# VIPL-Audio-Visual-Speech-Understanding/SBL_For_Multilingual_Lip_Reading

Hardware: AMD Instinct MI355X
Metric: lip-clips/sec fwd+bwd (29x88x88) (higher is better)
Workload: dtype f32 (exact 3-way bf16 split, 6 bf16 MFMA products per fp32 product, fp32 accumulate); 1 GPU; full SBL 6+6 (Conv3d stem + ResNet-18 + encoder + SBL decoder) fwd+loss+bwd (BASELINE config 3); matmul_precision=bf16x6, per_gpu_batch=32, global_batch=32, clip=29x88x88, parallelism=dp1, dropout=True, bn=train, issue=graph, hipgraph=True, decoder_streams=2, conv_weight_pack=cached (re-packed when weights change), decoder_schedule=teacher-forced runs batched, coin_patterns=8

## Files before the change

sbl_for_multilingual_lip_reading_amd/csrc/gemm.hip:

```cpp
#include <stdarg.h>
#include <stdlib.h>

#include <type_traits>
#include "mfma_gemm.h"
#include "skinny_gemm.h"

static thread_local char g_err[512] = "";
void sbl_set_error(const char* fmt, ...) {
    va_list ap;
    va_start(ap, fmt);
    vsnprintf(g_err, sizeof(g_err), fmt, ap);
    va_end(ap);
}
extern "C" const char* sbl_last_error(void) { return g_err; }

static unsigned long long* g_stamps = nullptr;
static int g_stamp_cap = 0, g_stamp_used = 0;
static thread_local int g_last_slot = -1, g_last_kid = 0;
unsigned long long* sbl_next_stamp_slot(int kernel_id) {
    g_last_kid = kernel_id;
    g_last_slot = -1;
    if (!g_stamps || g_stamp_used >= g_stamp_cap) return nullptr;
    g_last_slot = g_stamp_used++;
    return g_stamps + 2 * (size_t)g_last_slot;
}
extern "C" int sbl_profile_begin(uint64_t* stamps_dev, int capacity) {
    SBL_REQUIRE(stamps_dev && capacity > 0, "sbl_profile_begin: bad args");
    g_stamps = (unsigned long long*)stamps_dev;
    g_stamp_cap = capacity;
    g_stamp_used = 0;
    return 0;
}
extern "C" int sbl_profile_end(void) {
    const int used = g_stamp_used;
    g_stamps = nullptr;
    g_stamp_cap = g_stamp_used = 0;
    return used;
}
extern "C" int sbl_profile_last_slot(void) { return g_last_slot; }
extern "C" int sbl_profile_used(void) { return g_stamp_used; }
extern "C" int sbl_profile_last_kernel(void) { return g_last_kid; }
extern "C" int sbl_abi_version(void) { return SBL_ABI_VERSION; }

int g_sbl_prec = 0;
extern "C" int sbl_set_matmul_precision(int terms) {
    SBL_REQUIRE(terms == 0 || terms == 1 || terms == 3 || terms == 6,
                "sbl_set_matmul_precision: %d (0 = fp32 MFMA, 6 / 3 / 1 = split-bf16 MFMA terms)", terms);
    g_sbl_prec = terms;
    return 0;
}
extern "C" int sbl_get_matmul_precision(void) { return g_sbl_prec; }
int g_sbl_exp[8] = {0, 0, 0, 0, 0, 0, 0, 0};
int g_sbl_gemm2_split_target = 256, g_sbl_gemm2_split_max = 8;
int g_sbl_group_cap = 0;
int g_sbl_wave_ksplit = 1;
int g_sbl_ksplit_tiles = 320;
int g_sbl_big_min = 4096;
extern "C" int sbl_set_tuning(int knob, int value) {
    extern int g_sbl_wg_s2_small, g_sbl_wg_target, g_sbl_conv_patch;
    if (knob >= 100 && knob < 108) {
        g_sbl_exp[knob - 100] = value;
        return 0;
    }
    if (knob == 14) {
        extern int g_sbl_stem_fwd8;
        g_sbl_stem_fwd8 = value != 0;
        return 0;
    }
    if (knob == 13) {
        extern int g_sbl_stem_ablate;
        g_sbl_stem_ablate = value;
        return 0;
    }
    if (knob == 12) {
        extern int g_sbl_stem_wgrad_tr;
        g_sbl_stem_wgrad_tr = value != 0;
        return 0;
    }
    if (knob == 10 || knob == 11) {
        SBL_REQUIRE(value >= 1, "sbl_set_tuning: value < 1");
        (knob == 10 ? g_sbl_gemm2_split_target : g_sbl_gemm2_split_max) = value;
        return 0;
    }
    if (knob == 9) {
        extern int g_sbl_conv_patch_wgrad;
        SBL_REQUIRE(value >= 0, "sbl_set_tuning: negative value");
        g_sbl_conv_patch_wgrad = value;
        return 0;
    }
    if (knob == 8) {
        extern int g_sbl_conv_patch_imgs;
        SBL_REQUIRE(value >= 0, "sbl_set_tuning: negative value");
        g_sbl_conv_patch_imgs = value;
        return 0;
    }
    if (knob == 7) {
        extern int g_sbl_pm_wg64_maxm;
        SBL_REQUIRE(value >= 0, "sbl_set_tuning: negative value");
        g_sbl_pm_wg64_maxm = value;
        return 0;
    }
    if (knob == 6) {
        SBL_REQUIRE(value >= 0, "sbl_set_tuning: negative value");
        g_sbl_group_cap = value;
        return 0;
    }
    if (knob >= 3 && knob <= 5) {
        SBL_REQUIRE(value >= 0, "sbl_set_tuning: negative value");
        (knob == 3 ? g_sbl_wg_s2_small : knob == 4 ? g_sbl_wg_target : g_sbl_conv_patch) = value;
        return 0;
    }
    SBL_REQUIRE(knob >= 0 && knob <= 2 && value >= 0, "sbl_set_tuning: unknown knob %d / value %d (0 = wave-group K split on/off, 1 = 64x64-tile count from which dense products take 128x128 tiles, 2 = largest tile count that takes the wave-group K split)", knob, value);
    if (knob == 0) g_sbl_wave_ksplit = value != 0;
    else if (knob == 1) g_sbl_big_min = value;
    else g_sbl_ksplit_tiles = value;
    return 0;
}

template <class AL, class BL, int BM, int BN, int KU>
static void launch_mode(const AL& al, const BL& bl, float* C, long ldc, const float* bias, int relu,
                        const float* relu_mask, long ldm, int mode, int M, int N, int K, int splits, SplitCtl sc,
                        hipStream_t s) {
    if (mode == 0) {
        EpiStore<0, false> e{C, ldc, bias, relu, nullptr, relu_mask, ldm};
        sbl_launch_gemm<AL, BL, EpiStore<0, false>, BM, BN, KU>(al, bl, e, M, N, K, splits, s, sc);
    } else if (mode == 1) {
        EpiStore<1, false> e{C, ldc, bias, relu, nullptr, relu_mask, ldm};
        sbl_launch_gemm<AL, BL, EpiStore<1, false>, BM, BN, KU>(al, bl, e, M, N, K, splits, s, sc);
    } else {
        EpiStore<2, false> e{C, ldc, nullptr, 0, nullptr, nullptr, 0};
        sbl_launch_gemm<AL, BL, EpiStore<2, false>, BM, BN, KU>(al, bl, e, M, N, K, splits, s, sc);
    }
}

template <bool VEC, int BM, int BN, int KU>
static void launch_trans(int transA, int transB, const float* A, long lda, const float* B, long ldb, float* C, long ldc,
                         const float* bias, int relu, const float* relu_mask, long ldm, int mode, int M, int N, int K,
                         int splits, SplitCtl sc, hipStream_t s) {
    if (!transA && transB) {
        DenseKC<BM, VEC> al{A, lda, M};
        DenseKC<BN, VEC> bl{B, ldb, N};
        launch_mode<DenseKC<BM, VEC>, DenseKC<BN, VEC>, BM, BN, KU>(al, bl, C, ldc, bias, relu, relu_mask, ldm, mode, M, N, K, splits, sc, s);
    } else if (!transA && !transB) {
        DenseKC<BM, VEC> al{A, lda, M};
        DenseMC<BN, VEC> bl{B, ldb, N};
        launch_mode<DenseKC<BM, VEC>, DenseMC<BN, VEC>, BM, BN, KU>(al, bl, C, ldc, bias, relu, relu_mask, ldm, mode, M, N, K, splits, sc, s);
    } else if (transA && !transB) {
        DenseMC<BM, VEC> al{A, lda, M};
        DenseMC<BN, VEC> bl{B, ldb, N};
        launch_mode<DenseMC<BM, VEC>, DenseMC<BN, VEC>, BM, BN, KU>(al, bl, C, ldc, bias, relu, relu_mask, ldm, mode, M, N, K, splits, sc, s);
    } else {
        DenseMC<BM, VEC> al{A, lda, M};
        DenseKC<BN, VEC> bl{B, ldb, N};
        launch_mode<DenseMC<BM, VEC>, DenseKC<BN, VEC>, BM, BN, KU>(al, bl, C, ldc, bias, relu, relu_mask, ldm, mode, M, N, K, splits, sc, s);
    }
}

#define SBL_WS_COUNTERS 4096

extern "C" int sbl_gemm_f32(int transA, int transB, int M, int N, int K, const float* A, long lda, const float* B,
                            long ldb, float* C, long ldc, const float* bias, int relu, const float* relu_mask, long ldm,
                            int accumulate, float* a_colsum, void* ws, long ws_bytes, sbl_stream_t stream) {
    hipStream_t s = (hipStream_t)stream;
    SBL_REQUIRE(M > 0 && N > 0 && K > 0, "sbl_gemm_f32: non-positive dims M=%d N=%d K=%d", M, N, K);
    SBL_REQUIRE(A && B && C, "sbl_gemm_f32: null operand");
    SBL_REQUIRE(lda >= (transA ? M : K) && ldb >= (transB ? K : N) && ldc >= N,
                "sbl_gemm_f32: leading dimension too small (lda=%ld ldb=%ld ldc=%ld)", lda, ldb, ldc);
    SBL_REQUIRE(!relu_mask || ldm >= N, "sbl_gemm_f32: ldm=%ld < N=%d", ldm, N);
    SBL_REQUIRE(!a_colsum || transA, "sbl_gemm_f32: a_colsum needs transA=1 (A stored [K][M])");
    SBL_REQUIRE(!ws || (sbl_aligned16(ws) && ws_bytes >= (long)sizeof(int) * SBL_WS_COUNTERS), "sbl_gemm_f32: workspace unaligned or < 16 KiB");
    bool vec = sbl_aligned16(A) && sbl_aligned16(B) && (lda % 4 == 0) && (ldb % 4 == 0);
    if (!transA || transB) vec = vec && (K % 4 == 0);
    if (transA) vec = vec && (M % 4 == 0);
    if (!transB) vec = vec && (N % 4 == 0);
    SBL_REQUIRE(sbl_fits_u32((transA ? (long)K : (long)M) * lda) && sbl_fits_u32((transB ? (long)N : (long)K) * ldb),
                "sbl_gemm_f32: operand spans more than 2 GiB (buffer descriptor range)");
    const bool plain = !bias && !relu && !relu_mask;
    const long tiles64 = (long)sbl_cdiv(M, 64) * sbl_cdiv(N, 64);
    const int big_min = g_sbl_big_min;
    const bool big = (M >= 1024 && N >= 256 && tiles64 >= big_min);
    int splits = 1;
    constexpr int split_tiles = 192;
    constexpr int split_target = 256;
    if (!big && tiles64 < split_tiles && K >= 128) {
        splits = (int)((split_target + tiles64 - 1) / tiles64);
        if (splits > K / 64) splits = K / 64;
        if (splits > 8) splits = 8;
        if (splits < 1) splits = 1;
    }
    SplitCtl sc{nullptr, nullptr, a_colsum, nullptr};
    int mode = accumulate ? 1 : 0;
    if (splits > 1) {
        const long need = (long)sizeof(int) * SBL_WS_COUNTERS + tiles64 * splits * (long)(64 * 64 * sizeof(float));
        if (ws && tiles64 < SBL_WS_COUNTERS && need <= ws_bytes) {
            sc.counters = (int*)ws;
            sc.slabs = (float*)((char*)ws + sizeof(int) * SBL_WS_COUNTERS);
        } else if (plain) {
            mode = 2;
            if (!accumulate) SBL_HIP(hipMemset2DAsync(C, ldc * sizeof(float), 0, (size_t)N * sizeof(float), M, s));
        } else {
            splits = 1;
        }
    }
    {
        const bool a_kc = !transA, b_kc = transB != 0;
        const bool al_ok = (!a_kc || (sbl_aligned16(A) && lda % 4 == 0)) && (!b_kc || (sbl_aligned16(B) && ldb % 4 == 0));
        const bool k_ok = (!a_kc && !b_kc) || (K % 8 == 0);
        const long tiles32 = (long)sbl_cdiv(M, 32) * sbl_cdiv(N, 32);
        constexpr int max_m = 512;
        constexpr int max_t = 2048;
        constexpr int sq_rows = 1536;
        const bool shape_ok = transA ? ((K <= max_m && tiles32 <= max_t) || ((long)M * N <= 512L * 512 && K <= sq_rows))
                                     : ((M <= max_m && tiles32 <= max_t) || ((long)N * K <= 512L * 512 && M <= sq_rows));
        if (shape_ok && al_ok && k_ok && !(transA && transB)) {
            SkinnyEpi e{C, ldc, bias, relu, relu_mask, ldm, accumulate, a_colsum, sbl_next_stamp_slot(SBL_KID_SKINNY)};
            if (!transA && transB) sbl_launch_skinny<true, true>(A, lda, B, ldb, e, M, N, K, s);
            else if (!transA && !transB) sbl_launch_skinny<true, false>(A, lda, B, ldb, e, M, N, K, s);
            else sbl_launch_skinny<false, false>(A, lda, B, ldb, e, M, N, K, s);
            SBL_LAUNCH_CHECK("sbl_gemm_f32(skinny)");
            return 0;
        }
    }
    sc.stamp = sbl_next_stamp_slot(big ? SBL_KID_TILED128 : SBL_KID_TILED64);
#define SBL_GO(VEC, BM, BN, KU) \
    launch_trans<VEC, BM, BN, KU>(transA, transB, A, lda, B, ldb, C, ldc, bias, relu, relu_mask, ldm, mode, M, N, K, splits, sc, s)
    if (big) {
        constexpr int big_ku = 1;
        if (vec && big_ku == 2) SBL_GO(true, 128, 128, 2);
        else if (vec) SBL_GO(true, 128, 128, 1);
        else SBL_GO(false, 128, 128, 1);
    } else {
        constexpr int ku_env = 0;
        const int ku = ku_env ? ku_env : (tiles64 * splits > 512 ? 2 : 4);
        if (!vec) SBL_GO(false, 64, 64, 1);
        else if (ku == 1) SBL_GO(true, 64, 64, 1);
        else if (ku == 2) SBL_GO(true, 64, 64, 2);
        else SBL_GO(true, 64, 64, 4);
    }
#undef SBL_GO
    SBL_LAUNCH_CHECK("sbl_gemm_f32");
    return 0;
}

extern "C" int sbl_gemm2_f32(int M, int N, int K, const float* A0, const float* A1, long lda, const float* B0, const float* B1,
                             long ldb, float* C0, float* C1, long ldc, const float* bias0, const float* bias1, int relu,
                             void* ws, long ws_bytes, sbl_stream_t stream) {
    hipStream_t s = (hipStream_t)stream;
    SBL_REQUIRE(M > 0 && N > 0 && K > 0, "sbl_gemm2_f32: non-positive dims M=%d N=%d K=%d", M, N, K);
    SBL_REQUIRE(A0 && A1 && B0 && B1 && C0 && C1 && (!bias0 == !bias1), "sbl_gemm2_f32: null operand / one-sided bias");
    SBL_REQUIRE(lda >= K && ldb >= K && ldc >= N, "sbl_gemm2_f32: leading dimension too small (lda=%ld ldb=%ld ldc=%ld)", lda, ldb, ldc);
    SBL_REQUIRE(!ws || (sbl_aligned16(ws) && ws_bytes >= (long)sizeof(int) * SBL_WS_COUNTERS), "sbl_gemm2_f32: workspace unaligned or < 16 KiB");
    const bool vec = sbl_aligned16(A0) && sbl_aligned16(A1) && sbl_aligned16(B0) && sbl_aligned16(B1) && lda % 4 == 0 && ldb % 4 == 0 && K % 8 == 0;
    SBL_REQUIRE(sbl_fits_u32((long)M * lda) && sbl_fits_u32((long)N * ldb), "sbl_gemm2_f32: operand spans more than 2 GiB (buffer descriptor range)");
    const long tiles64 = (long)sbl_cdiv(M, 64) * sbl_cdiv(N, 64);
    const int big_min = g_sbl_big_min;
    const bool big = (M >= 1024 && N >= 256 && 2 * tiles64 >= big_min);
    if (!vec || big) {
        if (int e = sbl_gemm_f32(0, 1, M, N, K, A0, lda, B0, ldb, C0, ldc, bias0, relu, nullptr, 0, 0, nullptr, ws, ws_bytes, stream)) return e;
        return sbl_gemm_f32(0, 1, M, N, K, A1, lda, B1, ldb, C1, ldc, bias1, relu, nullptr, 0, 0, nullptr, ws, ws_bytes, stream);
    }
    {
        const long tiles32 = (long)sbl_cdiv(M, 32) * sbl_cdiv(N, 32);
        constexpr int max_m = 128;
        constexpr int max_t = 2048;
        constexpr int sq_rows = 768;
        if ((M <= max_m && tiles32 <= max_t) || ((long)N * K <= 512L * 512 && M <= sq_rows)) {
            SkinnyEpi e{C0, ldc, bias0, relu, nullptr, 0, 0, nullptr, sbl_next_stamp_slot(SBL_KID_SKINNY)};
            SkinnyDual du{A1, B1, C1, bias1};
            sbl_launch_skinny<true, true>(A0, lda, B0, ldb, e, M, N, K, s, &du);
            SBL_LAUNCH_CHECK("sbl_gemm2_f32(skinny)");
            return 0;
        }
    }
    int splits = 1;
    const int split_tiles = g_sbl_exp[1] > 0 ? g_sbl_exp[1] : 192;
    const int split_target = g_sbl_gemm2_split_target;
    if (2 * tiles64 < split_tiles && K >= 128) {
        splits = (int)((split_target + 2 * tiles64 - 1) / (2 * tiles64));
        if (splits > K / 64) splits = K / 64;
        if (splits > g_sbl_gemm2_split_max) splits = g_sbl_gemm2_split_max;
        if (splits < 1) splits = 1;
    }
    SplitCtl sc{nullptr, nullptr, nullptr, nullptr};
    if (splits > 1) {
        const long need = (long)sizeof(int) * SBL_WS_COUNTERS + 2 * tiles64 * splits * (long)(64 * 64 * sizeof(float));
        if (ws && 2 * tiles64 < SBL_WS_COUNTERS && need <= ws_bytes) {
            sc.counters = (int*)ws;
            sc.slabs = (float*)((char*)ws + sizeof(int) * SBL_WS_COUNTERS);
        } else {
            splits = 1;
        }
    }
    sc.stamp = sbl_next_stamp_slot(SBL_KID_TILED64);
    DenseKC<64, true> al{A0, lda, M};
    DenseKC<64, true> bl{B0, ldb, N};
    EpiStore<0, false> e{C0, ldc, bias0, relu, nullptr, nullptr, 0};
    GemmDual du{A1, B1, C1, bias1};
    constexpr int ku_env = 0;
    const int ku = ku_env ? ku_env : (2 * tiles64 * splits > 512 ? 2 : 4);
    if (ku == 2) sbl_launch_gemm2<DenseKC<64, true>, DenseKC<64, true>, EpiStore<0, false>, 64, 64, 2>(al, bl, e, du, M, N, K, splits, s, sc);
    else sbl_launch_gemm2<DenseKC<64, true>, DenseKC<64, true>, EpiStore<0, false>, 64, 64, 4>(al, bl, e, du, M, N, K, splits, s, sc);
    SBL_LAUNCH_CHECK("sbl_gemm2_f32");
    return 0;
}

extern "C" int sbl_wgrad_seg_f32(int nseg, const float* const* A_ptrs, long lda, const float* const* B_ptrs, long ldb,
                                 const int* seg_rows, int M, int N, float* C, long ldc, float* a_colsum,
                                 sbl_stream_t stream) {
    hipStream_t s = (hipStream_t)stream;
    SBL_REQUIRE(nseg >= 1 && nseg <= SBL_MAX_KSEG && A_ptrs && B_ptrs && seg_rows && C, "sbl_wgrad_seg_f32: bad segment list (nseg=%d)", nseg);
    SBL_REQUIRE(M > 0 && N > 0 && lda >= M && ldb >= N && ldc >= N && lda % 4 == 0 && ldb % 4 == 0, "sbl_wgrad_seg_f32: bad dims M=%d N=%d lda=%ld ldb=%ld", M, N, lda, ldb);
    constexpr int seg_tile_env = 0;
    constexpr int seg_ku = 2;
    constexpr int seg_target = 768;
    long K = 0;
    bool aligned = true;
    for (int t = 0; t < nseg; ++t) {
        aligned = aligned && (seg_rows[t] % SBL_BK == 0);
        SBL_REQUIRE(A_ptrs[t] && B_ptrs[t] && seg_rows[t] > 0 && sbl_aligned16(A_ptrs[t]) && sbl_aligned16(B_ptrs[t]), "sbl_wgrad_seg_f32: segment %d null/unaligned/empty", t);
        K += seg_rows[t];
    }
    SBL_REQUIRE(K < (1L << 30), "sbl_wgrad_seg_f32: too many rows");
    unsigned long long* stamp = sbl_next_stamp_slot(SBL_KID_SEG_WGRAD);
    auto go = [&](auto al, auto tile_c, auto ku_c) {
        constexpr int T = decltype(tile_c)::value, KUc = decltype(ku_c)::value;
        decltype(al) bl;
        long kc = 0;
        for (int t = 0; t < SBL_MAX_KSEG; ++t) {
            al.kcum[t] = bl.kcum[t] = (int)kc;
            al.p[t] = t < nseg ? A_ptrs[t] : nullptr;
            bl.p[t] = t < nseg ? B_ptrs[t] : nullptr;
            if (t < nseg) kc += seg_rows[t];
        }
        al.kcum[SBL_MAX_KSEG] = bl.kcum[SBL_MAX_KSEG] = (int)K;
        al.nseg = bl.nseg = nseg;
        al.ld = lda; bl.ld = ldb;
        al.rows = M; bl.rows = N;
        const long tiles = (long)sbl_cdiv(M, T) * sbl_cdiv(N, T);
        int splits = (int)((seg_target + tiles - 1) / tiles);
        if (splits > K / 128) splits = (int)(K / 128);
        if (splits < 1) splits = 1;
        EpiStore<2, false> e{C, ldc, nullptr, 0, nullptr, nullptr, 0};
        SplitCtl sc{nullptr, nullptr, a_colsum, stamp};
        sbl_launch_gemm<decltype(al), decltype(al), EpiStore<2, false>, T, T, KUc>(al, bl, e, M, N, (int)K, splits, s, sc);
    };
    using std::integral_constant;
    const int seg_tile = seg_tile_env ? seg_tile_env : ((long)sbl_cdiv(M, 128) * sbl_cdiv(N, 128) >= 48 ? 128 : 64);
    if (!aligned) go(SegMC<64, false>{}, integral_constant<int, 64>{}, integral_constant<int, 2>{});
    else if (seg_tile == 128) go(SegMC<128, true>{}, integral_constant<int, 128>{}, integral_constant<int, 1>{});
    else if (seg_ku == 4) go(SegMC<64, true>{}, integral_constant<int, 64>{}, integral_constant<int, 4>{});
    else go(SegMC<64, true>{}, integral_constant<int, 64>{}, integral_constant<int, 2>{});
    SBL_LAUNCH_CHECK("sbl_wgrad_seg_f32");
    return 0;
}

struct GroupProb {
    const float* a[SBL_MAX_KSEG];
    const float* b[SBL_MAX_KSEG];
    float* C;
    float* colsum;
    long lda, ldb, ldc;
    int M, N, tile0, tiles_m;
};
#define SBL_GROUP_WRITE 8
struct GroupWrite {
    GroupProb p[SBL_GROUP_WRITE];
};
__global__ void group_write_kernel(GroupWrite w, GroupProb* table, int first, int count) {
    const int i = threadIdx.x;
    if (i < count) table[first + i] = w.p[i];
}
struct GroupCommon {
    int nprob, nseg, K, ntiles;
    int kcum[SBL_MAX_KSEG + 1];
};
template <bool ONESEG, int PREC>
__global__ __launch_bounds__(256) void sbl_wgrad_group_kernel(const GroupProb* __restrict__ table, GroupCommon gc,
                                                              unsigned long long* stamp) {
  for (int t = blockIdx.x; t < gc.ntiles; t += gridDim.x) {
    if (t != (int)blockIdx.x) __syncthreads();
    int lo = 0, hi = gc.nprob - 1;
    while (lo < hi) {
        const int mid = (lo + hi + 1) >> 1;
        if (table[mid].tile0 <= t) lo = mid; else hi = mid - 1;
    }
    const GroupProb& g = table[lo];
    const int lt = t - g.tile0;
    const int tx = lt % g.tiles_m, ty = lt / g.tiles_m;
    EpiStore<1, false> e{g.C, g.ldc, nullptr, 0, nullptr, nullptr, 0};
    SplitCtl sc{nullptr, nullptr, g.colsum, stamp};
    if (ONESEG) {
        DenseMC<128, true> al{g.a[0], g.lda, g.M}, bl{g.b[0], g.ldb, g.N};
        sbl_gemm_tile<DenseMC<128, true>, DenseMC<128, true>, EpiStore<1, false>, 128, 128, 1, 2, PREC>(al, bl, e, sc, g.M, g.N, tx * 128,
                                                                                                    ty * 128, 0, gc.K, 0, 0, 1, ty == 0);
    } else {
        SegMC<128, true> al, bl;
#pragma unroll
        for (int s = 0; s < SBL_MAX_KSEG; ++s) {
            al.p[s] = g.a[s];
            bl.p[s] = g.b[s];
            al.kcum[s] = bl.kcum[s] = gc.kcum[s];
        }
        al.kcum[SBL_MAX_KSEG] = bl.kcum[SBL_MAX_KSEG] = gc.K;
        al.nseg = bl.nseg = gc.nseg;
        al.ld = g.lda; bl.ld = g.ldb;
        al.rows = g.M; bl.rows = g.N;
        sbl_gemm_tile<SegMC<128, true>, SegMC<128, true>, EpiStore<1, false>, 128, 128, 1, 2, PREC>(al, bl, e, sc, g.M, g.N, tx * 128,
                                                                                                  ty * 128, 0, gc.K, 0, 0, 1, ty == 0);
    }
  }
}

extern "C" long sbl_wgrad_group_table_bytes(int nprob) { return (long)sizeof(GroupProb) * (nprob > 0 ? nprob : 0); }

extern "C" int sbl_wgrad_group_f32(int nprob, int nseg, const int* seg_rows, const float* const* A_ptrs, const long* lda,
                                   const float* const* B_ptrs, const long* ldb, const int* M, const int* N, float* const* C,
                                   const long* ldc, float* const* colsum, void* table, long table_bytes,
                                   sbl_stream_t stream) {
    hipStream_t s = (hipStream_t)stream;
    SBL_REQUIRE(nprob >= 1 && nprob <= 4096 && nseg >= 1 && nseg <= SBL_MAX_KSEG && seg_rows && A_ptrs && B_ptrs && lda && ldb && M && N && C && ldc && colsum,
                "sbl_wgrad_group_f32: bad arguments (nprob=%d nseg=%d)", nprob, nseg);
    SBL_REQUIRE(table && sbl_aligned16(table) && table_bytes >= sbl_wgrad_group_table_bytes(nprob), "sbl_wgrad_group_f32: descriptor table too small");
    GroupCommon gc;
    gc.nprob = nprob;
    gc.nseg = nseg;
    long K = 0;
    for (int t = 0; t < SBL_MAX_KSEG; ++t) {
        gc.kcum[t] = (int)K;
        if (t < nseg) {
            SBL_REQUIRE(seg_rows[t] > 0 && seg_rows[t] % SBL_BK == 0, "sbl_wgrad_group_f32: segment %d has %d rows (must be a positive multiple of %d)", t, seg_rows[t], SBL_BK);
            K += seg_rows[t];
        }
    }
    SBL_REQUIRE(K < (1L << 30), "sbl_wgrad_group_f32: too many rows");
    gc.kcum[SBL_MAX_KSEG] = (int)K;
    gc.K = (int)K;
    long tiles = 0;
    GroupProb* tab = (GroupProb*)table;
    for (int first = 0; first < nprob; first += SBL_GROUP_WRITE) {
        GroupWrite w;
        const int count = nprob - first < SBL_GROUP_WRITE ? nprob - first : SBL_GROUP_WRITE;
        for (int i = 0; i < count; ++i) {
            const int p = first + i;
            GroupProb& g = w.p[i];
            SBL_REQUIRE(M[p] % 4 == 0 && N[p] % 4 == 0 && sbl_fits_u32(K * lda[p]) && sbl_fits_u32(K * ldb[p]),
                        "sbl_wgrad_group_f32: problem %d: M=%d / N=%d must be multiples of 4 and the operands at most 2 GiB", p, M[p], N[p]);
            SBL_REQUIRE(M[p] > 0 && N[p] > 0 && C[p] && lda[p] >= M[p] && ldb[p] >= N[p] && ldc[p] >= N[p] && lda[p] % 4 == 0 && ldb[p] % 4 == 0,
                        "sbl_wgrad_group_f32: problem %d has bad dims M=%d N=%d lda=%ld ldb=%ld ldc=%ld", p, M[p], N[p], lda[p], ldb[p], ldc[p]);
            for (int t = 0; t < SBL_MAX_KSEG; ++t) {
                g.a[t] = t < nseg ? A_ptrs[(long)p * nseg + t] : nullptr;
                g.b[t] = t < nseg ? B_ptrs[(long)p * nseg + t] : nullptr;
                SBL_REQUIRE(t >= nseg || (g.a[t] && g.b[t] && sbl_aligned16(g.a[t]) && sbl_aligned16(g.b[t])), "sbl_wgrad_group_f32: problem %d segment %d null/unaligned", p, t);
            }
            g.C = C[p];
            g.colsum = colsum[p];
            g.lda = lda[p]; g.ldb = ldb[p]; g.ldc = ldc[p];
            g.M = M[p]; g.N = N[p];
            g.tile0 = (int)tiles;
            g.tiles_m = sbl_cdiv(M[p], 128);
            tiles += (long)g.tiles_m * sbl_cdiv(N[p], 128);
        }
        hipLaunchKernelGGL(group_write_kernel, dim3(1), dim3(64), 0, s, w, tab, first, count);
    }
    SBL_REQUIRE(tiles < (1L << 30), "sbl_wgrad_group_f32: too many tiles");
    gc.ntiles = (int)tiles;
    if (g_sbl_group_cap > 0 && tiles > g_sbl_group_cap) tiles = g_sbl_group_cap;
#define SBL_KG1_(P) sbl_wgrad_group_kernel<true, P>
#define SBL_KG0_(P) sbl_wgrad_group_kernel<false, P>
    if (nseg == 1)
        SBL_PREC_LAUNCH(SBL_KG1_, dim3((unsigned)tiles), s, (const GroupProb*)tab, gc, sbl_next_stamp_slot(SBL_KID_SEG_WGRAD));
    else
        SBL_PREC_LAUNCH(SBL_KG0_, dim3((unsigned)tiles), s, (const GroupProb*)tab, gc, sbl_next_stamp_slot(SBL_KID_SEG_WGRAD));
#undef SBL_KG1_
#undef SBL_KG0_
    SBL_LAUNCH_CHECK("sbl_wgrad_group_f32");
    return 0;
}

__global__ __launch_bounds__(256) void colsum_kernel(const float* __restrict__ X, long ldx, float* __restrict__ out,
                                                     int M, int N, int rows_per_block) {
    __shared__ float red[4][64];
    const int c = blockIdx.x * 64 + (threadIdx.x & 63);
    const int rg = threadIdx.x >> 6;
    const int r0 = blockIdx.y * rows_per_block;
    const int r1 = min(M, r0 + rows_per_block);
    float s = 0.f;
    if (c < N)
        for (int r = r0 + rg; r < r1; r += 4) s += X[(long)r * ldx + c];
    red[rg][threadIdx.x & 63] = s;
    __syncthreads();
    if (rg == 0 && c < N) atomicAdd(out + c, red[0][threadIdx.x] + red[1][threadIdx.x] + red[2][threadIdx.x] + red[3][threadIdx.x]);
}

extern "C" int sbl_colsum_f32(const float* X, long ldx, float* out, int M, int N, int accumulate, sbl_stream_t stream) {
    hipStream_t s = (hipStream_t)stream;
    SBL_REQUIRE(M > 0 && N > 0 && X && out && ldx >= N, "sbl_colsum_f32: bad args M=%d N=%d ldx=%ld", M, N, ldx);
    if (!accumulate) SBL_HIP(hipMemsetAsync(out, 0, (size_t)N * sizeof(float), s));
    int gy = sbl_cdiv(M, 64);
    if (gy > 64) gy = 64;
    int rpb = sbl_cdiv(M, gy);
    hipLaunchKernelGGL(colsum_kernel, dim3(sbl_cdiv(N, 64), gy), dim3(256), 0, s, X, ldx, out, M, N, rpb);
    SBL_LAUNCH_CHECK("sbl_colsum_f32");
    return 0;
}
```

sbl_for_multilingual_lip_reading_amd/csrc/skinny_gemm.h:

```cpp
#pragma once
#include "sbl_common.h"

template <bool KCONTIG>
struct SkinnyOperand {
    const float* p;
    long ld;
    int rows;
    __device__ __forceinline__ float4 load(int r, int kb, int kend) const {
        float4 v = make_float4(0.f, 0.f, 0.f, 0.f);
        if (KCONTIG) {
            if (kb < kend) v = *reinterpret_cast<const float4*>(p + (long)r * ld + kb);
        } else {
            const float* q = p + (long)kb * ld + r;
            if (kb + 0 < kend) v.x = q[0];
            if (kb + 1 < kend) v.y = q[ld];
            if (kb + 2 < kend) v.z = q[2 * ld];
            if (kb + 3 < kend) v.w = q[3 * ld];
        }
        return v;
    }
};

struct SkinnyEpi {
    float* C;
    long ldc;
    const float* bias;
    int relu;
    const float* relu_mask;
    long ldm;
    int accumulate;
    float* a_colsum;
    unsigned long long* stamp;
};

struct SkinnyDual {
    const float* A1;
    const float* B1;
    float* C1;
    const float* bias1;
};

template <bool AKC, bool BKC, int NW, int U>
__global__ __launch_bounds__(NW * 64) void sbl_skinny_gemm_kernel(SkinnyOperand<AKC> a, SkinnyOperand<BKC> b, SkinnyEpi e,
                                                                  SkinnyDual du, int M, int N, int K) {
    __shared__ float red[NW][1024];
    __shared__ float csum[NW][32];
    if (blockIdx.z) {
        a.p = du.A1;
        b.p = du.B1;
        e.C = du.C1;
        e.bias = du.bias1;
    }
    const int tid = threadIdx.x, lane = tid & 63, wave = tid >> 6;
    const int i31 = lane & 31, h = lane >> 5;
    int mt = blockIdx.x, nt = blockIdx.y;
    {
        const int MT = gridDim.x, NT = gridDim.y;
        if ((NT & 7) == 0) {
            const int b = blockIdx.y * MT + blockIdx.x;
            const int xcd = b & 7, q = b >> 3;
            mt = q % MT;
            nt = (q / MT) * 8 + xcd;
        }
    }
    const int m0 = mt * 32, n0 = nt * 32;
    const int ra = min(m0 + i31, M - 1);
    const int rb = min(n0 + i31, N - 1);
    const int per = ((K + NW - 1) / NW + 7) & ~7;
    const int kbeg = wave * per;
    const int kend = min(K, kbeg + per);
    sbl_stamp_begin(e.stamp);

    f32x16 acc;
#pragma unroll
    for (int r = 0; r < 16; ++r) acc[r] = 0.f;
    float asum = 0.f;
    const bool do_colsum = e.a_colsum != nullptr && nt == 0;

    float4 a0[U], b0[U], a1[U], b1[U];
#define SK_LOAD(AV, BV, KB)                                   \
    _Pragma("unroll") for (int u = 0; u < U; ++u) {           \
        AV[u] = a.load(ra, (KB) + u * 8 + 4 * h, kend);       \
        BV[u] = b.load(rb, (KB) + u * 8 + 4 * h, kend);       \
    }
#define SK_MMA(AV, BV)                                                              \
    _Pragma("unroll") for (int u = 0; u < U; ++u) {                                 \
        const float4 x = AV[u], y = BV[u];                                          \
        acc = __builtin_amdgcn_mfma_f32_32x32x2f32(x.x, y.x, acc, 0, 0, 0);         \
        acc = __builtin_amdgcn_mfma_f32_32x32x2f32(x.y, y.y, acc, 0, 0, 0);         \
        acc = __builtin_amdgcn_mfma_f32_32x32x2f32(x.z, y.z, acc, 0, 0, 0);         \
        acc = __builtin_amdgcn_mfma_f32_32x32x2f32(x.w, y.w, acc, 0, 0, 0);         \
        if (do_colsum) asum += (x.x + x.y) + (x.z + x.w);                           \
    }
    SK_LOAD(a0, b0, kbeg)
    for (int k0 = kbeg; k0 < kend; k0 += 16 * U) {
        const bool has1 = k0 + 8 * U < kend;
        if (has1) { SK_LOAD(a1, b1, k0 + 8 * U) }
        SK_MMA(a0, b0)
        if (k0 + 16 * U < kend) { SK_LOAD(a0, b0, k0 + 16 * U) }
        if (has1) { SK_MMA(a1, b1) }
    }
#undef SK_LOAD
#undef SK_MMA
#pragma unroll
    for (int r = 0; r < 16; ++r) red[wave][r * 64 + lane] = acc[r];
    if (do_colsum) {
        asum += __shfl_xor(asum, 32, 64);
        if (h == 0) csum[wave][i31] = asum;
    }
    __syncthreads();
    if (do_colsum && tid < 32 && m0 + tid < M) {
        float s = 0.f;
#pragma unroll
        for (int w = 0; w < NW; ++w) s += csum[w][tid];
        atomicAdd(e.a_colsum + m0 + tid, s);
    }
    for (int el = tid; el < 1024; el += NW * 64) {
        float v = 0.f;
#pragma unroll
        for (int w = 0; w < NW; ++w) v += red[w][el];
        const int r = el >> 6, ln = el & 63;
        const int m = m0 + (r & 3) + 8 * (r >> 2) + 4 * (ln >> 5);
        const int n = n0 + (ln & 31);
        if (m < M && n < N) {
            if (e.bias) v += e.bias[n];
            if (e.relu) v = fmaxf(v, 0.f);
            if (e.relu_mask) v = e.relu_mask[(long)m * e.ldm + n] > 0.f ? v : 0.f;
            float* q = e.C + (long)m * e.ldc + n;
            if (e.accumulate) v += *q;
            *q = v;
        }
    }
    sbl_stamp_end(e.stamp);
}

template <bool AKC, bool BKC>
static inline void sbl_launch_skinny(const float* A, long lda, const float* B, long ldb, const SkinnyEpi& e, int M, int N,
                                     int K, hipStream_t s, const SkinnyDual* dual = nullptr) {
    SkinnyOperand<AKC> a{A, lda, M};
    SkinnyOperand<BKC> b{B, ldb, N};
    const SkinnyDual du = dual ? *dual : SkinnyDual{nullptr, nullptr, nullptr, nullptr};
    dim3 grid(sbl_cdiv(M, 32), sbl_cdiv(N, 32), dual ? 2 : 1);
    if (K >= 1024) hipLaunchKernelGGL((sbl_skinny_gemm_kernel<AKC, BKC, 8, 8>), grid, dim3(512), 0, s, a, b, e, du, M, N, K);
    else if (K >= 512) hipLaunchKernelGGL((sbl_skinny_gemm_kernel<AKC, BKC, 8, 4>), grid, dim3(512), 0, s, a, b, e, du, M, N, K);
    else hipLaunchKernelGGL((sbl_skinny_gemm_kernel<AKC, BKC, 4, 4>), grid, dim3(256), 0, s, a, b, e, du, M, N, K);
}
```

Measured before the change: 1024 clips/s.

## Add split-K slicing and bf16x6 MFMA path to dual skinny GEMM

The dual (two-GEMM) skinny path now splits K across extra workgroups when the tile count is small, writing per-slice partials to workspace slabs. A per-tile atomic counter lets the last-arriving block reduce them and run the epilogue. The same path can also use split-bf16 MFMA products at the configured precision instead of fp32 MFMA. The epilogue is restructured to batch its loads. This targets low occupancy and the slow fp32 MFMA on small decoder GEMMs, at the cost of extra workspace traffic and a serialized reduction.

```diff
diff --git a/sbl_for_multilingual_lip_reading_amd/csrc/gemm.hip b/sbl_for_multilingual_lip_reading_amd/csrc/gemm.hip
--- a/sbl_for_multilingual_lip_reading_amd/csrc/gemm.hip
+++ b/sbl_for_multilingual_lip_reading_amd/csrc/gemm.hip
@@ -157,6 +157,16 @@
 }
 
 #define SBL_WS_COUNTERS 4096
+
+static SkinnySplit skinny_split(long tiles, int K, void* ws, long ws_bytes) {
+    constexpr int target = 256, kmin = 128;
+    int kc = K;
+    const int nsl = sbl_skinny_slices(tiles, K, target, kmin, &kc);
+    const long need = (long)sizeof(int) * SBL_WS_COUNTERS + tiles * nsl * (long)(SBL_SKINNY_SLAB * sizeof(float));
+    if (nsl > 1 && ws && tiles < SBL_WS_COUNTERS && need <= ws_bytes)
+        return SkinnySplit{(float*)((char*)ws + sizeof(int) * SBL_WS_COUNTERS), (int*)ws, nsl, kc};
+    return SkinnySplit{nullptr, nullptr, 1, K};
+}
 
 extern "C" int sbl_gemm_f32(int transA, int transB, int M, int N, int K, const float* A, long lda, const float* B,
                             long ldb, float* C, long ldc, const float* bias, int relu, const float* relu_mask, long ldm,
@@ -214,9 +224,10 @@
                                      : ((M <= max_m && tiles32 <= max_t) || ((long)N * K <= 512L * 512 && M <= sq_rows));
         if (shape_ok && al_ok && k_ok && !(transA && transB)) {
             SkinnyEpi e{C, ldc, bias, relu, relu_mask, ldm, accumulate, a_colsum, sbl_next_stamp_slot(SBL_KID_SKINNY)};
-            if (!transA && transB) sbl_launch_skinny<true, true>(A, lda, B, ldb, e, M, N, K, s);
-            else if (!transA && !transB) sbl_launch_skinny<true, false>(A, lda, B, ldb, e, M, N, K, s);
-            else sbl_launch_skinny<false, false>(A, lda, B, ldb, e, M, N, K, s);
+            const SkinnySplit sp{nullptr, nullptr, 1, K};
+            if (!transA && transB) sbl_launch_skinny<true, true>(A, lda, B, ldb, e, M, N, K, s, nullptr, sp, 0);
+            else if (!transA && !transB) sbl_launch_skinny<true, false>(A, lda, B, ldb, e, M, N, K, s, nullptr, sp, 0);
+            else sbl_launch_skinny<false, false>(A, lda, B, ldb, e, M, N, K, s, nullptr, sp, 0);
             SBL_LAUNCH_CHECK("sbl_gemm_f32(skinny)");
             return 0;
         }
@@ -267,7 +278,7 @@
         if ((M <= max_m && tiles32 <= max_t) || ((long)N * K <= 512L * 512 && M <= sq_rows)) {
             SkinnyEpi e{C0, ldc, bias0, relu, nullptr, 0, 0, nullptr, sbl_next_stamp_slot(SBL_KID_SKINNY)};
             SkinnyDual du{A1, B1, C1, bias1};
-            sbl_launch_skinny<true, true>(A0, lda, B0, ldb, e, M, N, K, s, &du);
+            sbl_launch_skinny<true, true>(A0, lda, B0, ldb, e, M, N, K, s, &du, skinny_split(2 * tiles32, K, ws, ws_bytes), g_sbl_prec);
             SBL_LAUNCH_CHECK("sbl_gemm2_f32(skinny)");
             return 0;
         }
diff --git a/sbl_for_multilingual_lip_reading_amd/csrc/skinny_gemm.h b/sbl_for_multilingual_lip_reading_amd/csrc/skinny_gemm.h
--- a/sbl_for_multilingual_lip_reading_amd/csrc/skinny_gemm.h
+++ b/sbl_for_multilingual_lip_reading_amd/csrc/skinny_gemm.h
@@ -1,5 +1,6 @@
 #pragma once
 #include "sbl_common.h"
+#include "bf16_split.h"
 
 template <bool KCONTIG>
 struct SkinnyOperand {
@@ -40,12 +41,44 @@
     const float* bias1;
 };
 
-template <bool AKC, bool BKC, int NW, int U>
+typedef __attribute__((address_space(1))) float sbl_gfloat;
+#define SBL_SKINNY_SLAB 1056
+struct SkinnySplit {
+    float* slabs;
+    int* counters;
+    int nsl;
+    int kchunk;
+};
+
+template <int NT>
+__device__ __forceinline__ void sbl_skinny_bf_block(f32x16& acc, const float4& x0, const float4& x1, const float4& y0,
+                                                    const float4& y1) {
+    using T = BfTerms<NT>;
+    constexpr int NPL = T::NPL;
+    uint2 pa0[NPL], pa1[NPL], pb0[NPL], pb1[NPL];
+    bf_split4<NPL>(x0, pa0);
+    bf_split4<NPL>(x1, pa1);
+    bf_split4<NPL>(y0, pb0);
+    bf_split4<NPL>(y1, pb1);
+    bf16x8 a[NPL], b[NPL];
+#pragma unroll
+    for (int p = 0; p < NPL; ++p) {
+        a[p] = __builtin_bit_cast(bf16x8, make_uint4(pa0[p].x, pa0[p].y, pa1[p].x, pa1[p].y));
+        b[p] = __builtin_bit_cast(bf16x8, make_uint4(pb0[p].x, pb0[p].y, pb1[p].x, pb1[p].y));
+    }
+#pragma unroll
+    for (int t = 0; t < T::N; ++t) acc = __builtin_amdgcn_mfma_f32_32x32x16_bf16(a[T::pa(t)], b[T::pb(t)], acc, 0, 0, 0);
+}
+
+template <bool AKC, bool BKC, int NW, int U, int PREC>
 __global__ __launch_bounds__(NW * 64) void sbl_skinny_gemm_kernel(SkinnyOperand<AKC> a, SkinnyOperand<BKC> b, SkinnyEpi e,
-                                                                  SkinnyDual du, int M, int N, int K) {
+                                                                  SkinnyDual du, SkinnySplit sp, int M, int N, int K) {
+    static_assert(PREC == 0 || U % 2 == 0, "the bf16 body pairs 8-deep groups");
     __shared__ float red[NW][1024];
     __shared__ float csum[NW][32];
-    if (blockIdx.z) {
+    __shared__ int s_last;
+    const int dir = blockIdx.z / sp.nsl, slice = blockIdx.z - dir * sp.nsl;
+    if (dir) {
         a.p = du.A1;
         b.p = du.B1;
         e.C = du.C1;
@@ -66,9 +99,10 @@
     const int m0 = mt * 32, n0 = nt * 32;
     const int ra = min(m0 + i31, M - 1);
     const int rb = min(n0 + i31, N - 1);
-    const int per = ((K + NW - 1) / NW + 7) & ~7;
-    const int kbeg = wave * per;
-    const int kend = min(K, kbeg + per);
+    const int sbeg = slice * sp.kchunk, send = min(K, sbeg + sp.kchunk);
+    const int per = ((send - sbeg + NW - 1) / NW + 7) & ~7;
+    const int kbeg = sbeg + wave * per;
+    const int kend = min(send, kbeg + per);
     sbl_stamp_begin(e.stamp);
 
     f32x16 acc;
@@ -83,14 +117,25 @@
         AV[u] = a.load(ra, (KB) + u * 8 + 4 * h, kend);       \
         BV[u] = b.load(rb, (KB) + u * 8 + 4 * h, kend);       \
     }
-#define SK_MMA(AV, BV)                                                              \
-    _Pragma("unroll") for (int u = 0; u < U; ++u) {                                 \
-        const float4 x = AV[u], y = BV[u];                                          \
-        acc = __builtin_amdgcn_mfma_f32_32x32x2f32(x.x, y.x, acc, 0, 0, 0);         \
-        acc = __builtin_amdgcn_mfma_f32_32x32x2f32(x.y, y.y, acc, 0, 0, 0);         \
-        acc = __builtin_amdgcn_mfma_f32_32x32x2f32(x.z, y.z, acc, 0, 0, 0);         \
-        acc = __builtin_amdgcn_mfma_f32_32x32x2f32(x.w, y.w, acc, 0, 0, 0);         \
-        if (do_colsum) asum += (x.x + x.y) + (x.z + x.w);                           \
+#define SK_MMA(AV, BV)                                                                      \
+    if constexpr (PREC == 0) {                                                              \
+        _Pragma("unroll") for (int u = 0; u < U; ++u) {                                     \
+            const float4 x = AV[u], y = BV[u];                                              \
+            acc = __builtin_amdgcn_mfma_f32_32x32x2f32(x.x, y.x, acc, 0, 0, 0);             \
+            acc = __builtin_amdgcn_mfma_f32_32x32x2f32(x.y, y.y, acc, 0, 0, 0);             \
+            acc = __builtin_amdgcn_mfma_f32_32x32x2f32(x.z, y.z, acc, 0, 0, 0);             \
+            acc = __builtin_amdgcn_mfma_f32_32x32x2f32(x.w, y.w, acc, 0, 0, 0);             \
+            if (do_colsum) asum += (x.x + x.y) + (x.z + x.w);                               \
+        }                                                                                   \
+    } else {                                                                                \
+        _Pragma("unroll") for (int u = 0; u < U; u += 2) {                                  \
+            sbl_skinny_bf_block<PREC>(acc, AV[u], AV[u + 1], BV[u], BV[u + 1]);             \
+            if (do_colsum) {                                                                \
+                const float4 x = AV[u], z = AV[u + 1];                                      \
+                asum += (x.x + x.y) + (x.z + x.w);                                          \
+                asum += (z.x + z.y) + (z.z + z.w);                                          \
+            }                                                                               \
+        }                                                                                   \
     }
     SK_LOAD(a0, b0, kbeg)
     for (int k0 = kbeg; k0 < kend; k0 += 16 * U) {
@@ -109,39 +154,128 @@
         if (h == 0) csum[wave][i31] = asum;
     }
     __syncthreads();
-    if (do_colsum && tid < 32 && m0 + tid < M) {
-        float s = 0.f;
-#pragma unroll
-        for (int w = 0; w < NW; ++w) s += csum[w][tid];
-        atomicAdd(e.a_colsum + m0 + tid, s);
-    }
-    for (int el = tid; el < 1024; el += NW * 64) {
-        float v = 0.f;
-#pragma unroll
-        for (int w = 0; w < NW; ++w) v += red[w][el];
+    constexpr int PER_T = 1024 / (NW * 64);
+    float v[PER_T];
+#pragma unroll
+    for (int j = 0; j < PER_T; ++j) {
+        const int el = tid + j * NW * 64;
+        v[j] = 0.f;
+#pragma unroll
+        for (int w = 0; w < NW; ++w) v[j] += red[w][el];
+    }
+    float cs = 0.f;
+    if (do_colsum && tid < 32) {
+#pragma unroll
+        for (int w = 0; w < NW; ++w) cs += csum[w][tid];
+    }
+    if (sp.nsl > 1) {
+        const int tile = (dir * gridDim.y + nt) * gridDim.x + mt;
+        float* mine = sp.slabs + ((long)tile * sp.nsl + slice) * SBL_SKINNY_SLAB;
+#pragma unroll
+        for (int j = 0; j < PER_T; ++j)
+            __hip_atomic_store((sbl_gfloat*)mine + tid + j * NW * 64, v[j], __ATOMIC_RELAXED, __HIP_MEMORY_SCOPE_AGENT);
+        if (do_colsum && tid < 32) __hip_atomic_store((sbl_gfloat*)mine + 1024 + tid, cs, __ATOMIC_RELAXED, __HIP_MEMORY_SCOPE_AGENT);
+        asm volatile("s_waitcnt vmcnt(0)" ::: "memory");
+        __syncthreads();
+        if (tid == 0) {
+            const int t = __hip_atomic_fetch_add(sp.counters + tile, 1, __ATOMIC_RELAXED, __HIP_MEMORY_SCOPE_AGENT);
+            const int last = (t == sp.nsl - 1);
+            if (last) __hip_atomic_store(sp.counters + tile, 0, __ATOMIC_RELAXED, __HIP_MEMORY_SCOPE_AGENT);
+            s_last = last;
+        }
+        __syncthreads();
+        if (!s_last) {
+            sbl_stamp_end(e.stamp);
+            return;
+        }
+        __builtin_amdgcn_fence(__ATOMIC_ACQUIRE, "wavefront");
+        const sbl_gfloat* base = (const sbl_gfloat*)sp.slabs + (long)tile * sp.nsl * SBL_SKINNY_SLAB;
+#pragma unroll
+        for (int j = 0; j < PER_T; ++j) v[j] = 0.f;
+        cs = 0.f;
+        for (int z = 0; z < sp.nsl; ++z) {
+            const sbl_gfloat* q = base + (long)z * SBL_SKINNY_SLAB;
+            float t[PER_T];
+#pragma unroll
+            for (int j = 0; j < PER_T; ++j) t[j] = __hip_atomic_load(q + tid + j * NW * 64, __ATOMIC_RELAXED, __HIP_MEMORY_SCOPE_AGENT);
+#pragma unroll
+            for (int j = 0; j < PER_T; ++j) v[j] += t[j];
+            if (do_colsum && tid < 32) cs += __hip_atomic_load(q + 1024 + tid, __ATOMIC_RELAXED, __HIP_MEMORY_SCOPE_AGENT);
+        }
+    }
+    if (do_colsum && tid < 32 && m0 + tid < M) atomicAdd(e.a_colsum + m0 + tid, cs);
+    long off[PER_T], moff[PER_T];
+    int col[PER_T];
+    bool in[PER_T];
+    float bv[PER_T], mv[PER_T], cv[PER_T];
+#pragma unroll
+    for (int j = 0; j < PER_T; ++j) {
+        const int el = tid + j * NW * 64;
         const int r = el >> 6, ln = el & 63;
         const int m = m0 + (r & 3) + 8 * (r >> 2) + 4 * (ln >> 5);
         const int n = n0 + (ln & 31);
-        if (m < M && n < N) {
-            if (e.bias) v += e.bias[n];
-            if (e.relu) v = fmaxf(v, 0.f);
-            if (e.relu_mask) v = e.relu_mask[(long)m * e.ldm + n] > 0.f ? v : 0.f;
-            float* q = e.C + (long)m * e.ldc + n;
-            if (e.accumulate) v += *q;
-            *q = v;
-        }
+        in[j] = m < M && n < N;
+        col[j] = min(n, N - 1);
+        off[j] = (long)min(m, M - 1) * e.ldc + col[j];
+        moff[j] = (long)min(m, M - 1) * e.ldm + col[j];
+    }
+#pragma unroll
+    for (int j = 0; j < PER_T; ++j) bv[j] = 0.f, mv[j] = 1.f, cv[j] = 0.f;
+    if (e.bias) {
+#pragma unroll
+        for (int j = 0; j < PER_T; ++j) bv[j] = e.bias[col[j]];
+    }
+    if (e.relu_mask) {
+#pragma unroll
+        for (int j = 0; j < PER_T; ++j) mv[j] = e.relu_mask[moff[j]];
+    }
+    if (e.accumulate) {
+#pragma unroll
+        for (int j = 0; j < PER_T; ++j) cv[j] = e.C[off[j]];
+    }
+#pragma unroll
+    for (int j = 0; j < PER_T; ++j) {
+        float x = v[j];
+        if (e.bias) x += bv[j];
+        if (e.relu) x = fmaxf(x, 0.f);
+        if (e.relu_mask) x = mv[j] > 0.f ? x : 0.f;
+        if (e.accumulate) x += cv[j];
+        if (in[j]) e.C[off[j]] = x;
     }
     sbl_stamp_end(e.stamp);
+}
+
+static inline int sbl_skinny_slices(long wgs, int K, int target, int kmin, int* kchunk) {
+    int nsl = (int)(target / (wgs > 0 ? wgs : 1));
+    const int kmax = K / (kmin > 32 ? kmin : 32);
+    if (nsl > kmax) nsl = kmax;
+    if (nsl > 16) nsl = 16;
+    if (nsl < (K >= 1024 ? 2 : 4)) nsl = 1;
+    const int kc = (sbl_cdiv(K, nsl) + 31) & ~31;
+    *kchunk = nsl > 1 ? kc : K;
+    return nsl > 1 ? sbl_cdiv(K, kc) : 1;
 }
 
 template <bool AKC, bool BKC>
 static inline void sbl_launch_skinny(const float* A, long lda, const float* B, long ldb, const SkinnyEpi& e, int M, int N,
-                                     int K, hipStream_t s, const SkinnyDual* dual = nullptr) {
+                                     int K, hipStream_t s, const SkinnyDual* dual, SkinnySplit sp, int prec) {
     SkinnyOperand<AKC> a{A, lda, M};
     SkinnyOperand<BKC> b{B, ldb, N};
     const SkinnyDual du = dual ? *dual : SkinnyDual{nullptr, nullptr, nullptr, nullptr};
-    dim3 grid(sbl_cdiv(M, 32), sbl_cdiv(N, 32), dual ? 2 : 1);
-    if (K >= 1024) hipLaunchKernelGGL((sbl_skinny_gemm_kernel<AKC, BKC, 8, 8>), grid, dim3(512), 0, s, a, b, e, du, M, N, K);
-    else if (K >= 512) hipLaunchKernelGGL((sbl_skinny_gemm_kernel<AKC, BKC, 8, 4>), grid, dim3(512), 0, s, a, b, e, du, M, N, K);
-    else hipLaunchKernelGGL((sbl_skinny_gemm_kernel<AKC, BKC, 4, 4>), grid, dim3(256), 0, s, a, b, e, du, M, N, K);
-}
+    if (sp.nsl <= 1) sp = SkinnySplit{nullptr, nullptr, 1, K};
+    dim3 grid(sbl_cdiv(M, 32), sbl_cdiv(N, 32), (dual ? 2 : 1) * sp.nsl);
+    const int kc = sp.kchunk;
+#define SK_GO(NW, U, P) hipLaunchKernelGGL((sbl_skinny_gemm_kernel<AKC, BKC, NW, U, P>), grid, dim3(NW * 64), 0, s, a, b, e, du, sp, M, N, K)
+#define SK_PREC(NW, U)                   \
+    switch (prec) {                      \
+        case 6: SK_GO(NW, U, 6); break;  \
+        case 3: SK_GO(NW, U, 3); break;  \
+        case 1: SK_GO(NW, U, 1); break;  \
+        default: SK_GO(NW, U, 0); break; \
+    }
+    if (kc >= 1024) { SK_PREC(8, 8) }
+    else if (kc >= 512) { SK_PREC(8, 4) }
+    else { SK_PREC(4, 4) }
+#undef SK_PREC
+#undef SK_GO
+}
```

Measured after the change: 1032 clips/s, median of 6. About the same (+0.9%).
